# lukeduball/VoxelRaymarcher

Hardware: NVIDIA B200
Metric: primary_mrays_per_s_4k_512cube (higher is better)
Workload: dtype f32

## Files before the change

__graft_entry__.py:

```python
from __future__ import annotations

import os
import subprocess
import sys

ROOT = os.path.dirname(os.path.abspath(__file__))
if ROOT not in sys.path:
    sys.path.insert(0, ROOT)


def _run(cmd):
    proc = subprocess.run(cmd, cwd=ROOT, stdout=subprocess.PIPE, stderr=subprocess.STDOUT, text=True)
    if proc.returncode != 0:
        raise RuntimeError(f"{' '.join(cmd)} failed:\n{proc.stdout[-4000:]}")
    return proc.stdout


def build() -> None:
    _run(["make", "-j4", "-C", os.path.join(ROOT, "voxelraymarcher_b200", "csrc")])
    _run(["make", "-C", os.path.join(ROOT, "oracle"), "port"])
    _run(["make", "-j3", "-C", os.path.join(ROOT, "oracle"), "ref"])
    _run(["make", "-C", os.path.join(ROOT, "tests", "hostsim")])
    import voxelraymarcher_b200
    from voxelraymarcher_b200 import api
    api.load_library()


def smoke() -> None:
    import numpy as np
    from voxelraymarcher_b200 import api, scenes
    from oracle import pyoracle as po

    if not api.device_available():
        raise RuntimeError("smoke() needs a CUDA device: the product has no CPU fallback")
    xyz, rgb = scenes.probe_scene()
    width, height = 320, 180
    cam = api.Camera((6.0, 2.0, 6.0), (0.0, 0.0, -1.0), (0.0, 1.0, 0.0), 60.0, np.float32(width) / np.float32(height))
    kind = "refh" if po.available("refh") else "orc"
    po.set_lighting(kind)
    for storage in ("hashtable", "vcs"):
        scene = api.VoxelScene(0)
        scene.add_voxels(xyz, rgb)
        scene.generate_voxel_scene(storage)
        ref = po.OracleScene(kind)
        ref.add_voxels(xyz, rgb)
# ... 21 lines not shown
```

include/vrm_b200.h:

```cpp
#ifndef VRM_B200_H
#define VRM_B200_H

#include <stdint.h>

#ifdef __cplusplus
extern "C" {
#endif

typedef struct vrm_scene vrm_scene;

enum
{
	VRM_OK = 0,
	VRM_ERR_INVALID = 1,
	VRM_ERR_CUDA = 2,
	VRM_ERR_STATE = 3,
	VRM_ERR_NOMEM = 4,
	VRM_ERR_BUILD = 5
};

enum { VRM_STORAGE_VCS = 0, VRM_STORAGE_HASHTABLE = 1 };
enum { VRM_ALGO_LONGEST_AXIS = 0, VRM_ALGO_ORIGINAL = 1 };

#define VRM_EMPTY (1u << 30)
// ... 58 lines not shown

#define VRM_IPC_HANDLE_BYTES 64
int vrm_peer_alloc(int device, uint64_t bytes, void** d_ptr_out, unsigned char handle_out[VRM_IPC_HANDLE_BYTES]);
int vrm_peer_open(int device, const unsigned char handle[VRM_IPC_HANDLE_BYTES], void** d_ptr_out);
int vrm_peer_close(int device, void* d_ptr);
int vrm_peer_free(int device, void* d_ptr);
int vrm_copy_device(int device, void* d_dst, const void* d_src, uint64_t bytes);

int vrm_scene_set_completion_flag(vrm_scene* scene, uint32_t* d_flag, uint32_t first_value);
int vrm_scene_set_completion_counter(vrm_scene* scene, uint32_t* d_counter);
int vrm_claim_next(int device, void* cuda_stream, uint32_t* d_counter, uint32_t* h_claimed);
int vrm_wait_flags_device(int device, void* cuda_stream, const uint32_t* d_flags, uint32_t n_flags, uint32_t stride_words,
                          uint32_t min_value, uint32_t timeout_ms, int* d_status);

int vrm_render_views_sharded(vrm_scene* const* scenes, uint32_t n_scenes, const float* cameras, uint32_t n_views,
                             const float translation[3], uint32_t scale, int algorithm, uint32_t width, uint32_t height,
                             uint8_t* rgb_out, int out_on_device, uint32_t* views_per_scene_out, float* total_ms);

int vrm_lookup(vrm_scene* scene, const int32_t* xyz, uint64_t n, uint32_t* out, uint8_t* exists_out);

int vrm_set_l2_persistence(vrm_scene* scene, int enabled);

int vrm_set_statistics(vrm_scene* scene, int enabled);
int vrm_get_statistics(vrm_scene* scene, uint64_t out[8]);

int vrm_microbench_l2(int device, uint64_t working_set_bytes, float* gather8_loads_per_ns, float* gather8_gbs, float* stream_gbs);

#ifdef __cplusplus
}
#endif
#endif
```

voxelraymarcher_b200/api.py:

```python
from __future__ import annotations

import ctypes as C
import os

import numpy as np

HERE = os.path.dirname(os.path.abspath(__file__))
LIB_PATH = os.environ.get("VRM_B200_LIB") or os.path.join(HERE, "libvrm_b200.so")

STORAGE_VCS, STORAGE_HASHTABLE = 0, 1
ALGO_LONGEST_AXIS, ALGO_ORIGINAL = 0, 1
STORAGE = {"vcs": STORAGE_VCS, "hashtable": STORAGE_HASHTABLE}
ALGORITHM = {"longestaxis": ALGO_LONGEST_AXIS, "original": ALGO_ORIGINAL}
EMPTY = 1 << 30

EXPORTS = [
    "vrm_error_string", "vrm_last_error", "vrm_device_available", "vrm_device_count", "vrm_device_name", "vrm_scene_create", "vrm_scene_destroy",
    "vrm_scene_set_stream", "vrm_scene_reset_stream", "vrm_scene_synchronize", "vrm_scene_add_voxels", "vrm_scene_add_voxels_device", "vrm_scene_insert_voxel",
    "vrm_scene_generate_terrain", "vrm_scene_generate_sparse_shells", "vrm_scene_generate_cube", "vrm_scene_generate_sphere",
    "vrm_scene_build", "vrm_scene_info", "vrm_set_lighting", "vrm_camera_make", "vrm_make_unit_vector", "vrm_render",
    "vrm_render_device", "vrm_render_views_device", "vrm_render_views_device_strided", "vrm_render_views", "vrm_trace_rays", "vrm_trace_rays_device", "vrm_lookup",
    "vrm_set_l2_persistence", "vrm_set_statistics", "vrm_get_statistics", "vrm_peer_alloc", "vrm_peer_open", "vrm_peer_close", "vrm_peer_free", "vrm_copy_device", "vrm_microbench_l2",
    "vrm_scene_set_completion_flag", "vrm_scene_set_completion_counter", "vrm_claim_next", "vrm_wait_flags_device", "vrm_render_views_sharded",
]


class VrmError(RuntimeError):
    pass


_lib = None


def load_library():
    global _lib
    if _lib is not None:
        return _lib
    if not os.path.exists(LIB_PATH):
        raise VrmError(f"{LIB_PATH} is missing: build it with `python -c 'import __graft_entry__ as g; g.build()'` "
                       "(there is no CPU fallback)")
    lib = C.CDLL(LIB_PATH)
    vp, u64, u32, i32, ci, f32 = C.c_void_p, C.c_uint64, C.c_uint32, C.c_int32, C.c_int, C.c_float
    sig = {
        "vrm_error_string": (C.c_char_p, [ci]),
        "vrm_last_error": (C.c_char_p, [vp]),
# ... 12 lines not shown
        "vrm_scene_generate_sparse_shells": (ci, [vp, u32, u32, u32, u32, C.POINTER(u64)]),
        "vrm_scene_generate_cube": (ci, [vp, i32, i32, i32, i32, C.POINTER(u64)]),
        "vrm_scene_generate_sphere": (ci, [vp, u32, u32, u32, u32, ci, C.POINTER(u64)]),
        "vrm_scene_build": (ci, [vp, ci, C.POINTER(f32)]),
        "vrm_scene_info": (ci, [vp, C.POINTER(u32), C.POINTER(i32), C.POINTER(u32), C.POINTER(u64), C.POINTER(u64)]),
        "vrm_set_lighting": (ci, [vp, vp, vp, vp, ci, ci]),
        "vrm_camera_make": (ci, [vp, vp, vp, f32, f32, vp]),
        "vrm_make_unit_vector": (ci, [vp, vp]),
        "vrm_render": (ci, [vp, vp, vp, u32, ci, u32, u32, vp, vp, C.POINTER(f32)]),
        "vrm_render_device": (ci, [vp, vp, vp, u32, ci, u32, u32, vp, vp]),
        "vrm_render_views_device": (ci, [vp, vp, u32, vp, u32, ci, u32, u32, vp, vp]),
        "vrm_render_views_device_strided": (ci, [vp, vp, u32, vp, u32, ci, u32, u32, vp, vp, u32]),
        "vrm_render_views": (ci, [vp, vp, u32, vp, u32, ci, u32, u32, vp, C.POINTER(f32)]),
        "vrm_trace_rays": (ci, [vp, vp, u64, vp, u32, ci, vp, vp, C.POINTER(f32)]),
        "vrm_trace_rays_device": (ci, [vp, vp, u64, vp, u32, ci, vp, vp]),
        "vrm_lookup": (ci, [vp, vp, u64, vp, vp]),
        "vrm_peer_alloc": (ci, [ci, u64, C.POINTER(vp), vp]),
        "vrm_peer_open": (ci, [ci, vp, C.POINTER(vp)]),
        "vrm_peer_close": (ci, [ci, vp]),
        "vrm_peer_free": (ci, [ci, vp]),
        "vrm_copy_device": (ci, [ci, vp, vp, u64]),
        "vrm_set_l2_persistence": (ci, [vp, ci]),
        "vrm_set_statistics": (ci, [vp, ci]),
        "vrm_get_statistics": (ci, [vp, vp]),
        "vrm_microbench_l2": (ci, [ci, u64, C.POINTER(f32), C.POINTER(f32), C.POINTER(f32)]),
        "vrm_scene_set_completion_flag": (ci, [vp, vp, u32]),
        "vrm_scene_set_completion_counter": (ci, [vp, vp]),
        "vrm_claim_next": (ci, [ci, vp, vp, vp]),
        "vrm_wait_flags_device": (ci, [ci, vp, vp, u32, u32, u32, u32, vp]),
        "vrm_render_views_sharded": (ci, [vp, u32, vp, u32, vp, u32, ci, u32, u32, vp, ci, vp, C.POINTER(f32)]),
    }
    for name, (res, args) in sig.items():
        fn = getattr(lib, name)
        fn.restype = res
        fn.argtypes = args
    _lib = lib
    return lib


def device_available() -> bool:
    return bool(load_library().vrm_device_available())


def microbench_l2(device: int = 0, working_set_bytes: int = 32 << 20):
    a, b, c = C.c_float(), C.c_float(), C.c_float()
    rc = load_library().vrm_microbench_l2(device, working_set_bytes, C.byref(a), C.byref(b), C.byref(c))
# ... 196 lines not shown
                          translation=(0.0, 0.0, 0.0)):
        self._check(self.lib.vrm_trace_rays_device(self.h, C.c_void_p(d_rays_ptr), n, _ptr(_f3(translation)), scale, self._algo(algorithm),
                                                   C.c_void_p(d_colour_ptr), C.c_void_p(d_hits_ptr or 0)), "vrm_trace_rays_device")

    def lookup(self, xyz):
        xyz = np.ascontiguousarray(xyz, np.int32).reshape(-1, 3)
        n = xyz.shape[0]
        out = np.zeros(n, np.uint32)
        exists = np.zeros(n, np.uint8)
        self._check(self.lib.vrm_lookup(self.h, _ptr(xyz), n, _ptr(out), _ptr(exists)), "vrm_lookup")
        return out, exists

    def set_completion_flag(self, d_flag_ptr: int | None, first_value: int = 1):
        self._check(self.lib.vrm_scene_set_completion_flag(self.h, C.c_void_p(d_flag_ptr or 0), first_value), "vrm_scene_set_completion_flag")

    def set_completion_counter(self, d_counter_ptr: int | None):
        self._check(self.lib.vrm_scene_set_completion_counter(self.h, C.c_void_p(d_counter_ptr or 0)), "vrm_scene_set_completion_counter")

    def set_l2_persistence(self, enabled: bool):
        self._check(self.lib.vrm_set_l2_persistence(self.h, int(enabled)), "vrm_set_l2_persistence")

    def set_statistics(self, enabled: bool, as_executed: bool = False):
        self._check(self.lib.vrm_set_statistics(self.h, (2 if as_executed else 1) if enabled else 0), "vrm_set_statistics")

    def get_statistics(self):
        out = np.zeros(8, np.uint64)
        self._check(self.lib.vrm_get_statistics(self.h, _ptr(out)), "vrm_get_statistics")
        keys = ["exist_checks", "exist_false", "lookups", "lookup_hits", "table2_probes", "region_reads", "rays", "crawl_skipped"]
        return {k: int(v) for k, v in zip(keys, out)}


def render_views_sharded(scene_list, width, height, algorithm, cameras, scale=1, translation=(0.0, 0.0, 0.0), rgb_out=None, d_rgb_ptr: int | None = None):
    lib = load_library()
    cams = np.ascontiguousarray(np.stack([VoxelScene._cam(c) for c in cameras]).astype(np.float32))
    n = cams.shape[0]
    handles = (C.c_void_p * len(scene_list))(*[s.h for s in scene_list])
    counts = np.zeros(len(scene_list), np.uint32)
    ms = C.c_float()
    on_device = d_rgb_ptr is not None
    if not on_device:
        if rgb_out is None:
            rgb_out = np.zeros((n, height, width, 3), np.uint8)
        assert rgb_out.dtype == np.uint8 and rgb_out.size == n * height * width * 3 and rgb_out.flags["C_CONTIGUOUS"]
    out = C.c_void_p(d_rgb_ptr) if on_device else _ptr(rgb_out)
    rc = lib.vrm_render_views_sharded(C.cast(handles, C.c_void_p), len(scene_list), _ptr(cams), n, _ptr(_f3(translation)), int(scale),
                                      VoxelScene._algo(algorithm), width, height, out, int(on_device), _ptr(counts), C.byref(ms))
# ... 4 lines not shown
```

voxelraymarcher_b200/csrc/vrm_api.cu:

```cuda
#include "vrm_internal.h"
#include "../../include/vrm_b200.h"

#include <cmath>
#include <cstdlib>
#include <cstring>
#include <new>

using namespace vrm;

int vrm_fail_cuda(vrm_scene* s, cudaError_t e, const char* what)
{
	if (s) s->lastError = std::string(what) + ": " + cudaGetErrorString(e);
	cudaGetLastError();
	return e == cudaErrorMemoryAllocation ? VRM_ERR_NOMEM : VRM_ERR_CUDA;
}

void vrm_apply_l2_window(vrm_scene* s)
{
	const bool want = s->l2Persist && s->storage >= 0;
	if (want == s->l2WindowOn && (!want || s->l2WindowStream == s->stream)) return;
	cudaStreamAttrValue attr;
	memset(&attr, 0, sizeof(attr));
	if (s->l2WindowOn && s->l2WindowStream && s->l2WindowStream != s->stream)
	{
// ... 135 lines not shown
	s->device = device;
	float inv[3] = {1.0f, 1.0f, 1.0f};
	vrm_make_unit_vector(inv, s->light.dir);
	s->light.color[0] = s->light.color[1] = s->light.color[2] = 1.0f;
	s->light.pos[0] = 10.0f; s->light.pos[1] = 10.0f; s->light.pos[2] = -10.0f;
	s->light.usePoint = 0; s->light.useShadows = 1;
	cudaError_t e = cudaSetDevice(device);
	if (e == cudaSuccess) vrm_configure_pool(device);
	if (e == cudaSuccess) e = cudaStreamCreateWithFlags(&s->ownStream, cudaStreamNonBlocking);
	if (e == cudaSuccess) e = cudaEventCreate(&s->ev0);
	if (e == cudaSuccess) e = cudaEventCreate(&s->ev1);
	if (e == cudaSuccess) e = cudaMalloc(&s->d_stats, sizeof(Stats));
	if (e == cudaSuccess) e = cudaMemset(s->d_stats, 0, sizeof(Stats));
	if (e == cudaSuccess) e = cudaMalloc(&s->d_queue, sizeof(unsigned int));

	if (e == cudaSuccess) e = cudaDeviceGetAttribute(&s->numSms, cudaDevAttrMultiProcessorCount, device);
	if (const char* mode = getenv("VRM_RENDER_MODE")) s->renderMode = atoi(mode);
	if (const char* form = getenv("VRM_SHADOW_FORM")) { const int f = atoi(form); if (f >= 0 && f <= 2) s->shadowForm = f; }
	if (const char* lp = getenv("VRM_L2_PERSIST")) s->l2Persist = atoi(lp) != 0;
	if (const char* ts = getenv("VRM_TRACE_SORT")) s->traceSort = atoi(ts);
	if (const char* tf = getenv("VRM_TRACE_FUSED")) s->traceFused = atoi(tf);
	if (const char* pd = getenv("VRM_PINNED_DMA")) s->pinnedDma = atoi(pd);
	if (const char* ws = getenv("VRM_WSTORE_REMOTE")) s->wstoreRemote = atoi(ws) != 0;
	if (const char* bs = getenv("VRM_BULK_STORE")) s->bulkStore = atoi(bs) != 0;
	if (const char* bb = getenv("VRM_VIEW_BATCH_BYTES")) { long long v = atoll(bb); if (v > 0) s->viewBatchBytes = (size_t)v; }
	if (e != cudaSuccess) { vrm_scene_destroy(s); cudaGetLastError(); return VRM_ERR_CUDA; }
	s->stream = s->ownStream;
	cudaEventRecord(s->ev1, s->stream);
	*out = s;
	return VRM_OK;
}

int vrm_scene_destroy(vrm_scene* s)
{
	if (!s) return VRM_OK;
	cudaSetDevice(s->device);
	if (s->stream) cudaStreamSynchronize(s->stream);
	vrm_stage_free(s);
	vrm_free_async(s, s->d_regionMinMax); s->d_regionMinMax = nullptr;
	vrm_free_structure(s);
	cudaStreamSynchronize(s->stream);
	cudaFree(s->d_hits); cudaFree(s->d_cams); cudaFree(s->d_io); cudaFree(s->d_stats); cudaFree(s->d_queue); cudaFree(s->d_defer); cudaFree(s->d_parkBits); cudaFree(s->d_parkCtl); cudaFree(s->d_gather); cudaFree(s->d_shadowItems); cudaFree(s->d_shadowCtl); cudaFree(s->d_localFrame); if (s->h_stage) cudaFreeHost(s->h_stage); for (auto& e : s->evBand) if (e) cudaEventDestroy(e);
	if (s->h_cams) cudaFreeHost(s->h_cams);
	if (s->ev0) cudaEventDestroy(s->ev0);
	if (s->ev1) cudaEventDestroy(s->ev1);
	if (s->ownStream) cudaStreamDestroy(s->ownStream);
// ... 421 lines not shown
{
	if (!d_dst || !d_src) return VRM_ERR_INVALID;
	if (cudaSetDevice(device) != cudaSuccess || cudaMemcpy(d_dst, d_src, bytes, cudaMemcpyDeviceToDevice) != cudaSuccess) { cudaGetLastError(); return VRM_ERR_CUDA; }
	return VRM_OK;
}

int vrm_set_l2_persistence(vrm_scene* s, int enabled)
{
	if (!s) return VRM_ERR_INVALID;
	VRM_CUDA(s, cudaSetDevice(s->device));
	s->l2Persist = enabled != 0;
	vrm_apply_l2_window(s);
	return VRM_OK;
}

int vrm_set_statistics(vrm_scene* s, int enabled)
{
	if (!s) return VRM_ERR_INVALID;
	s->statsEnabled = enabled != 0;
	s->statsMode = enabled == 2 ? 2 : (enabled ? 1 : 0);
	return VRM_OK;
}

int vrm_get_statistics(vrm_scene* s, uint64_t out[8])
{
	if (!s || !out) return VRM_ERR_INVALID;
	VRM_CUDA(s, cudaSetDevice(s->device));
	Stats h;
	VRM_CUDA(s, cudaMemcpyAsync(&h, s->d_stats, sizeof(Stats), cudaMemcpyDeviceToHost, s->stream));
	VRM_CUDA(s, cudaStreamSynchronize(s->stream));
	out[0] = h.nExist; out[1] = h.nExistFalse; out[2] = h.nLookup; out[3] = h.nLookupHit; out[4] = h.nProbe2; out[5] = h.nRegionReads;
	out[6] = s->statsRays; out[7] = h.nCrawlSkipped;
	return VRM_OK;
}

}
```

voxelraymarcher_b200/csrc/vrm_build.cu:

```cuda
#include "vrm_internal.h"

#include <chrono>
#include <cstdio>
#include <cstdlib>
#include "../../include/vrm_b200.h"

#include <algorithm>

using namespace vrm;

namespace
{

constexpr int kThreads = 256;
constexpr int kSortItems = 8;
constexpr int kSortTile = kThreads * kSortItems;
constexpr int kMaxDigitBits = 9;
constexpr int kMaxBins = 1 << kMaxDigitBits;
constexpr int kScanItems = 8;
constexpr int kScanTile = kThreads * kScanItems;
constexpr int kMaxEvictions = 400;
constexpr int kMaxRebuilds = 24;
constexpr int kRoundsPerBatch = 3;

// ... 190 lines not shown
	cellOcc[cell] = 1u;
}

__global__ void counts_kernel(const uint32_t* __restrict__ pos, const uint32_t* __restrict__ keep, uint64_t n,
                              const uint32_t* __restrict__ cellRank, const uint32_t* __restrict__ cellOcc, uint64_t cells, uint32_t* __restrict__ counts)
{
	counts[0] = pos[n - 1] + keep[n - 1];
	counts[1] = cellRank[cells - 1] + cellOcc[cells - 1];
}

__global__ void region_table_kernel(const uint32_t* __restrict__ cellFirst, const uint32_t* __restrict__ cellRank, const uint32_t* __restrict__ cellOcc, uint64_t cells,
                                    uint32_t numRegions, uint32_t unique, int32_t* __restrict__ regionTable, uint32_t* __restrict__ regionStart)
{
	uint64_t c = blockIdx.x * (uint64_t)blockDim.x + threadIdx.x;
	if (c == 0) regionStart[numRegions] = unique;
	if (c >= cells) return;
	if (cellOcc[c])
	{
		const uint32_t ri = cellRank[c];
		regionTable[c] = (int32_t)ri;
		regionStart[ri] = cellFirst[c];
	}
	else regionTable[c] = -1;
}

template <class K>
__global__ void vcs_fill_kernel(const K* __restrict__ ukeys, const int32_t* __restrict__ regionTable, uint64_t u,
                                uint2* __restrict__ headers, uint32_t* __restrict__ clusterMask)
{
	uint64_t j = blockIdx.x * (uint64_t)blockDim.x + threadIdx.x;
	if (j >= u) return;
	K k = ukeys[j];
	if (j != 0 && (ukeys[j - 1] >> 5) == (k >> 5)) return;
	uint32_t ri = (uint32_t)regionTable[(uint64_t)(k >> 18)];
	uint32_t cid = (uint32_t)(k >> 9) & 511u, code = (uint32_t)k & 511u;
	uint32_t mask = 1u << (code & 31);
	for (uint64_t t = j + 1; t < u && t < j + 32; t++)
	{
		K kt = ukeys[t];
		if ((kt >> 5) != (k >> 5)) break;
		mask |= 1u << ((uint32_t)kt & 31);
	}
	headers[((size_t)ri * 512 + cid) * 16 + (code >> 5)] = make_uint2(mask, (uint32_t)j);
	bool firstOfCluster = j == 0 || (ukeys[j - 1] >> 9) != (k >> 9);
	if (firstOfCluster) atomicOr(clusterMask + (size_t)ri * 16 + (cid >> 5), 1u << (cid & 31));
}
// ... 186 lines not shown
		region_heads_kernel<K><<<grid_for(n), kThreads, 0, st>>>(kin, pos, n, cellFirst, cellOcc);
		exclusive_scan(cellOcc, cellRank, tableSize, scratch, st);
		counts_kernel<<<1, 1, 0, st>>>(pos, keep, n, cellRank, cellOcc, tableSize, counts);
		uint32_t hostCounts[2] = {0, 0};
		VRM_CUDA(s, cudaMemcpyAsync(hostCounts, counts, sizeof(hostCounts), cudaMemcpyDeviceToHost, st));
		VRM_CUDA(s, cudaStreamSynchronize(st));
		unique = hostCounts[0];
		numRegions = hostCounts[1];
		if (unique == n) { ukeys = kin; uvals = vin; valsAreStageRgb = vin == s->d_stageRgb; }
		else
		{
			if (uniq.alloc(pad256(unique * sizeof(K)) + unique * 4) != cudaSuccess) { cudaGetLastError(); s->lastError = "unique voxel allocation failed"; return VRM_ERR_NOMEM; }
			ukeys = uniq.as<K>();
			uvals = reinterpret_cast<uint32_t*>(uniq.as<char>() + pad256(unique * sizeof(K)));
			compact_kernel<K><<<grid_for(n), kThreads, 0, st>>>(kin, vin, keep, pos, n, ukeys, uvals);
		}
		trace.mark(st, "dedupe + region heads");
		if (regionStart.alloc(((size_t)numRegions + 1) * 4) != cudaSuccess) { cudaGetLastError(); s->lastError = "region directory allocation failed"; return VRM_ERR_NOMEM; }
		region_table_kernel<<<grid_for(tableSize), kThreads, 0, st>>>(cellFirst, cellRank, cellOcc, tableSize, numRegions, (uint32_t)unique, regionTable.as<int32_t>(), regionStart.as<uint32_t>());
		VRM_CUDA(s, cudaGetLastError());
		trace.mark(st, "region directory");
	}

	uint64_t bytes = tableSize * sizeof(int32_t);
	PoolBuf headers(s), clusterMask(s), hashDesc(s), slots(s), values(s);
	if (storageType == VRM_STORAGE_VCS)
	{
		constexpr size_t kGuardClusters = 80;
		const size_t headerGuard = kGuardClusters * 16 * sizeof(uint2), maskGuard = 128;
		const size_t headerBytes = (size_t)numRegions * 512 * 16 * sizeof(uint2);
		if (unique >= (1ull << 31) || ((uint64_t)numRegions * 512ull + kGuardClusters) * 16ull >= (1ull << 32)) { s->lastError = "scene too large for the VCS index widths"; return VRM_ERR_INVALID; }
		if (headers.alloc(headerBytes + headerGuard) != cudaSuccess || clusterMask.alloc((size_t)numRegions * 16 * 4 + maskGuard) != cudaSuccess)
		{ cudaGetLastError(); s->lastError = "VCS allocation failed"; return VRM_ERR_NOMEM; }
		VRM_CUDA(s, cudaMemsetAsync(headers.p, 0, headerBytes + headerGuard, st));
		VRM_CUDA(s, cudaMemsetAsync(clusterMask.p, 0, (size_t)numRegions * 16 * 4 + maskGuard, st));
		if (unique)
		{
			vcs_fill_kernel<K><<<grid_for(unique), kThreads, 0, st>>>(ukeys, regionTable.as<int32_t>(), unique, headers.as<uint2>(), clusterMask.as<uint32_t>());
			vcs_flag_clusters_kernel<<<grid_for((uint64_t)numRegions * 512), kThreads, 0, st>>>(headers.as<uint2>(), clusterMask.as<uint32_t>(), (uint64_t)numRegions * 512);
		}
		if (unique && valsAreStageRgb) { values.s = s; values.p = s->d_stageRgb; s->d_stageRgb = nullptr; }
		else
		{
			if (values.alloc(unique * 4) != cudaSuccess) { cudaGetLastError(); s->lastError = "colour array allocation failed"; return VRM_ERR_NOMEM; }
			if (unique) VRM_CUDA(s, cudaMemcpyAsync(values.p, uvals, unique * 4, cudaMemcpyDeviceToDevice, st));
		}
		VRM_CUDA(s, cudaGetLastError());
// ... 31 lines not shown
				for (; round < batchEnd; round++)
				{
					cuckoo_insert_kernel<K><<<grid_for(unique), kThreads, 0, st>>>(ukeys, uvals, regionTable.as<int32_t>(), unique, hashDesc.as<HashRegionDesc>(),
					                                                              slots.as<unsigned long long>(), retry, failed, failCount, round);
					cuckoo_round_end_kernel<<<numRegions, kThreads, 0, st>>>(slots.as<unsigned long long>(), hashDesc.as<HashRegionDesc>(), retry, failed, failCount, round);
				}
				uint32_t hostFail[kMaxRebuilds] = {};
				VRM_CUDA(s, cudaMemcpyAsync(hostFail, failCount, round * 4, cudaMemcpyDeviceToHost, st));
				VRM_CUDA(s, cudaStreamSynchronize(st));
				for (uint32_t r = 0; r < round; r++) if (hostFail[r] == 0u) converged = true;
				if (trace.on) for (uint32_t r = 0; r < round; r++) fprintf(stderr, "[vrm build] cuckoo round %u: %u regions failed\n", r, hostFail[r]);
			}
			if (!converged) { s->lastError = "cuckoo insertion did not converge"; return VRM_ERR_BUILD; }
			VRM_CUDA(s, cudaGetLastError());
		}
		bytes += (size_t)numRegions * sizeof(HashRegionDesc) + totalSlots * 8 + (size_t)numRegions * 64;
		trace.mark(st, "cuckoo insertion");
	}
	VRM_CUDA(s, cudaEventRecord(s->ev1, st));
	VRM_CUDA(s, cudaStreamSynchronize(st));
	VRM_CUDA(s, cudaGetLastError());

	s->d_regionTable = static_cast<int32_t*>(regionTable.release());
	if (storageType == VRM_STORAGE_VCS)
	{
		s->d_headers = static_cast<uint2*>(headers.release());
		s->d_clusterMask = static_cast<uint32_t*>(clusterMask.release());
		s->d_values = static_cast<uint32_t*>(values.release());
	}
	else
	{
		s->d_hashDesc = static_cast<HashRegionDesc*>(hashDesc.release());
		s->d_clusterMask = static_cast<uint32_t*>(clusterMask.release());
		s->d_slots = static_cast<unsigned long long*>(slots.release());
	}
	s->storage = storageType;
	s->diameter = (uint32_t)D;
	s->minCoord = minCoord;
	s->filled = numRegions;
	s->unique = unique;
	s->bytes = bytes;
	return VRM_OK;
}

}

// ... 63 lines not shown
	*d_xyz = s->d_stageXyz + s->nStaged * 3;
	*d_rgb = s->d_stageRgb + s->nStaged;
	return VRM_OK;
}

int vrm_stage_commit(vrm_scene* s, uint64_t n)
{
	if (n == 0) return VRM_OK;
	if (!s->d_regionMinMax)
	{
		cudaError_t e = vrm_alloc_async(s, reinterpret_cast<void**>(&s->d_regionMinMax), 2 * sizeof(int));
		if (e == cudaSuccess) e = cudaMemsetAsync(s->d_regionMinMax, 0, 2 * sizeof(int), s->stream);
		if (e != cudaSuccess) return vrm_fail_cuda(s, e, "region extent allocation");
	}
	region_minmax_kernel<<<(unsigned)std::min<uint64_t>((n * 3 + kThreads - 1) / kThreads, 148 * 16), kThreads, 0, s->stream>>>(s->d_stageXyz + s->nStaged * 3, n, s->d_regionMinMax);
	VRM_CUDA(s, cudaGetLastError());
	s->nStaged += n;
	return VRM_OK;
}

void vrm_free_structure(vrm_scene* s)
{
	vrm_free_async(s, s->d_regionTable); s->d_regionTable = nullptr;
	vrm_free_async(s, s->d_hashDesc); s->d_hashDesc = nullptr;
	vrm_free_async(s, s->d_slots); s->d_slots = nullptr;
	vrm_free_async(s, s->d_headers); s->d_headers = nullptr;
	vrm_free_async(s, s->d_clusterMask); s->d_clusterMask = nullptr;
	vrm_free_async(s, s->d_values); s->d_values = nullptr;
	s->storage = -1; s->bytes = 0; s->filled = 0; s->unique = 0;
}

int vrm_build_structure(vrm_scene* s, int storageType, float* buildMs)
{
	cudaStream_t st = s->stream;
	BuildTrace trace;
	VRM_CUDA(s, cudaEventRecord(s->ev0, st));
	int rc = vrm_stage_flush_pending(s);
	if (rc) return rc;
	int hostMinMax[2] = {0, 0};
	if (s->d_regionMinMax)
	{
		VRM_CUDA(s, cudaMemcpyAsync(hostMinMax, s->d_regionMinMax, sizeof(hostMinMax), cudaMemcpyDeviceToHost, st));
		VRM_CUDA(s, cudaStreamSynchronize(st));
	}
	trace.mark(st, "extent");
	const int minCoord = hostMinMax[0];
// ... 46 lines not shown
```

voxelraymarcher_b200/csrc/vrm_core.cuh:

```cuda
#pragma once

#ifndef VRM_SMEM_MASK
#define VRM_SMEM_MASK 0
#endif

#include <stdint.h>
#include <math.h>
#include <string.h>
#include <type_traits>

#if defined(__CUDACC__)
#define VRM_HD __host__ __device__ __forceinline__
#define VRM_HD_NOINLINE static __host__ __device__ __noinline__
#else
#define VRM_HD inline
#define VRM_HD_NOINLINE static inline
#endif

namespace vrm
{

constexpr float kEps = 0.0001f;
constexpr uint32_t kEmpty = 1u << 30;
constexpr uint32_t kContinue = kEmpty + 2u;
// ... 106 lines not shown

VRM_HD float div1(float x, const RayDir& k, int i)
{
	float ax = fabsf(x);
	if (!(ax >= k.thr)) return vdiv(x, k.d[i]);
	return div_by_const(x, k.d[i], k.rd[i]);
}


struct Lighting
{
	float dir[3];
	float color[3];
	float pos[3];
	int usePoint;
	int useShadows;
};

struct LightWalk
{
	float idD[3], idR[3], idThr;
	float laD[3], laR[3], laSD[3], laSR[3], laThr;
	uint32_t laPerm;
};

struct HashRegionDesc
{
	uint32_t slotBase;
	uint32_t n;
	uint32_t seed1, seed2;
};

struct SceneView
{
	const int32_t* regionTable;
	uint32_t diameter;
	int32_t minCoord;
	const HashRegionDesc* hashDesc;
	const unsigned long long* slots;
	const uint2* headers;
	const uint32_t* clusterMask;
	const uint32_t* values;
};

struct Stats
{
	unsigned long long nExist, nExistFalse, nLookup, nLookupHit, nProbe2, nRegionReads;
	unsigned long long nCrawlSkipped;
};


struct PermIdentity
{
	VRM_HD int axis(int i) const { return i; }
	VRM_HD int cs(int i) const { return 6 - 3 * i; }
	VRM_HD int ks(int i) const { return 14 - 7 * i; }
	VRM_HD uint32_t stride(int i, uint32_t D) const { return i == 0 ? 1u : (i == 1 ? D : D * D); }
};
// ... 208 lines not shown
	if (STATS) c.st.nLookup++;
	if (v != kEmpty) note_lookup_hit(c, p, reg, g0, g1, g2);
	return v;
}

template <int ST, bool STATS, class P>
VRM_HD void record_hit_voxel(RayCtx<ST, STATS>& c, const P& p, const int* reg, int g0, int g1, int g2)
{
	if (!c.hitOut) return;
	int gw[3] = {reg[0] * kRegion + g0, reg[1] * kRegion + g1, reg[2] * kRegion + g2};
	int gx[3];
	to_world(p, gw, gx);
	c.hitOut[0] = gx[0]; c.hitOut[1] = gx[1]; c.hitOut[2] = gx[2]; c.hitOut[3] = 1;
}

template <int ST, bool STATS, class P>
VRM_HD int32_t region_entry(RayCtx<ST, STATS>& c, const P& p, const int* reg)
{
	uint32_t D = c.sv.diameter;
	uint32_t u0 = (uint32_t)(reg[0] - c.sv.minCoord), u1 = (uint32_t)(reg[1] - c.sv.minCoord), u2 = (uint32_t)(reg[2] - c.sv.minCoord);
	if (!(u0 < D && u1 < D && u2 < D)) return -2;
	if (STATS) c.st.nRegionReads++;
	return ldg(c.sv.regionTable + (u0 * p.stride(0, D) + u1 * p.stride(1, D) + u2 * p.stride(2, D)));
}


VRM_HD uint32_t vec_to_rgb(float r, float g, float b)
{
	uint32_t ir = (uint32_t)vmul(r, 255.0f), ig = (uint32_t)vmul(g, 255.0f), ib = (uint32_t)vmul(b, 255.0f);
	return (ir << 16) | (ig << 8) | ib;
}

VRM_HD uint32_t apply_lighting(const Lighting& L, const float* translation, uint32_t voxelColor, int normalAxis, float normalSign,
                               const float* hitLocal, const int* regW)
{
	float cr = vdiv((float)(voxelColor >> 16), 255.0f);
	float cg = vdiv((float)((voxelColor >> 8) & 0xFF), 255.0f);
	float cb = vdiv((float)(voxelColor & 0xFF), 255.0f);
	float n[3] = {0.0f, 0.0f, 0.0f};
	n[0] = normalAxis == 0 ? normalSign : 0.0f;
	n[1] = normalAxis == 1 ? normalSign : 0.0f;
	n[2] = normalAxis == 2 ? normalSign : 0.0f;
	if (L.usePoint)
	{
		float t[3];
		for (int i = 0; i < 3; i++)
// ... 580 lines not shown
```

voxelraymarcher_b200/csrc/vrm_flat.cuh:

```cuda
#pragma once

#include "vrm_core.cuh"

#if defined(__CUDACC__)
#define VRM_FLAT_COLD __host__ __device__ __noinline__
#else
#define VRM_FLAT_COLD
#endif

#ifndef VRM_VCS_FUSED_EXIST
#define VRM_VCS_FUSED_EXIST 1
#endif

namespace vrm
{

enum FlatState : int
{
	kStMainLast = 4,
	kStRegion = 5,
	kStHead = 6,
	kStHit = 7,
	kStDone = 8,
	kStPark = 9
};

enum AdvMode : int
{
	kAdvNone = 0,
	kAdvNext = 1,
	kAdvCluster = 2,
	kAdvJump = 3,
	kAdvRegion = 4
};

constexpr uint32_t kFlShadow = 1u;
constexpr uint32_t kFlShadowLA = 2u;
constexpr uint32_t kFlEq0 = 4u;
constexpr uint32_t kFlEqMask = 28u;
constexpr int kFlPermShift = 8;
constexpr int32_t kRiPending = -3;

constexpr int kPpOff = 0, kPpDefer = 1, kPpInline = 2;
#ifndef VRM_REGION_VOTE
#define VRM_REGION_VOTE 0
#endif
#ifndef VRM_HEAD_VOTE
#define VRM_HEAD_VOTE 0
#endif
#ifndef VRM_PP_DEFAULT
#define VRM_PP_DEFAULT 2
#endif
#ifndef VRM_FAST_LA
#define VRM_FAST_LA 7
#endif
#ifndef VRM_CC_MUL
#define VRM_CC_MUL 1
#endif
#ifndef VRM_CLS_LUT
#define VRM_CLS_LUT 1
#endif
#ifndef VRM_FAST_ENTER
// ... 16 lines not shown

VRM_HD PermRuntime unpack_perm(uint32_t fl)
{
	PermRuntime p;
	p.a0 = (int)((fl >> kFlPermShift) & 3u); p.a1 = (int)((fl >> (kFlPermShift + 2)) & 3u); p.a2 = (int)((fl >> (kFlPermShift + 4)) & 3u);
	return p;
}
VRM_HD uint32_t pack_perm(const PermRuntime& p) { return ((uint32_t)p.a0 | ((uint32_t)p.a1 << 2) | ((uint32_t)p.a2 << 4)) << kFlPermShift; }

VRM_HD LightWalk make_light_walk(const Lighting& L)
{
	LightWalk w;
	const RayDir ki = make_raydir(L.dir[0], L.dir[1], L.dir[2]);
	for (int i = 0; i < 3; i++) { w.idD[i] = ki.d[i]; w.idR[i] = ki.rd[i]; }
	w.idThr = ki.thr;
	const PermRuntime p = rank_axes(L.dir[0], L.dir[1], L.dir[2]);
	float dw[3];
	to_walk(p, L.dir, dw);
	const RayDir k = make_raydir(dw[0], dw[1], dw[2]);
	const RayDir ko = scaled_raydir(k);
	for (int i = 0; i < 3; i++) { w.laD[i] = k.d[i]; w.laR[i] = k.rd[i]; w.laSD[i] = ko.d[i]; w.laSR[i] = ko.rd[i]; }
	w.laThr = (k.thr == k.thr && ko.thr == ko.thr) ? k.thr : NAN;
	w.laPerm = pack_perm(p);
	return w;
}

VRM_HD uint32_t apply_lighting_flat(const Lighting& L, const float* translation, uint32_t voxelColor, int normalAxis, float normalSign,
                                    const float* hitLocal, const int* regW)
{
	if (L.usePoint) return apply_lighting(L, translation, voxelColor, normalAxis, normalSign, hitLocal, regW);
	const float r255 = 0.00392156886f;
	const float cr = div_by_const((float)(voxelColor >> 16), 255.0f, r255);
	const float cg = div_by_const((float)((voxelColor >> 8) & 0xFF), 255.0f, r255);
	const float cb = div_by_const((float)(voxelColor & 0xFF), 255.0f, r255);
	const float n0 = normalAxis == 0 ? normalSign : 0.0f, n1 = normalAxis == 1 ? normalSign : 0.0f, n2 = normalAxis == 2 ? normalSign : 0.0f;
	const float diff = fmaxf(vadd(vadd(vmul(n0, L.dir[0]), vmul(n1, L.dir[1])), vmul(n2, L.dir[2])), 0.0f);
	return vec_to_rgb(vmul(cr, vmul(diff, L.color[0])), vmul(cg, vmul(diff, L.color[1])), vmul(cb, vmul(diff, L.color[2])));
}

VRM_HD void primary_ray_flat(const float* cam, uint32_t x, uint32_t y, uint32_t W, uint32_t H, float invW, float invH, float* o, float* d)
{
	const float u = div_by_const(vadd((float)x, 0.5f), (float)W, invW);
	const float v = div_by_const(vadd((float)(H - y), 0.5f), (float)H, invH);
	float rel[3];
	for (int i = 0; i < 3; i++)
	{
// ... 37 lines not shown
		st = kStDone;
	}

	VRM_HD void set_perm(const SceneView& sv, const PermRuntime& p)
	{
		fl = (fl & ~(63u << kFlPermShift)) | pack_perm(p);
		const uint32_t D = sv.diameter;
		const int a[3] = {p.a0, p.a1, p.a2};
		for (int i = 0; i < 3; i++)
		{
			sh[i] = ST == kStorageHash ? (uint32_t)(kHashKeyBits * (2 - a[i])) : (uint32_t)(6 - 3 * a[i]);
#if VRM_CC_MUL
			sh[i] = 1u << sh[i];
#endif
			rs[i] = a[i] == 0 ? 1u : (a[i] == 1 ? D : D * D);
		}
	}

	VRM_HD void read_region_entry(RayCtx<ST, STATS>& c)
	{
		const uint32_t D = c.sv.diameter;
		if (!(ur[0] < D && ur[1] < D && ur[2] < D)) { ri = -2; return; }
		if (STATS) c.st.nRegionReads++;
		ri = ldg(c.sv.regionTable + (ur[0] * rs[0] + ur[1] * rs[1] + ur[2] * rs[2]));
	}

	VRM_HD void change_region(RayCtx<ST, STATS>& c)
	{
		for (int i = 0; i < 3; i++)
		{
			const int diff = (int)floorf(vmul(o[i], 0.015625f));
			ur[i] += (uint32_t)diff;
			o[i] = vsub(o[i], (float)(diff * kRegion));
		}
		st = kStRegion;
		if (!position_sane(o)) { ri = -2; return; }
		read_region_entry(c);
	}

	VRM_HD void start_primary(RayCtx<ST, STATS>& c, const float* originW, const float* dirW, float scale)
	{
		fl = 0; result = 0; ri = -2; seq = 0; ad1 = ad2 = 0;
		g[0] = g[1] = g[2] = 0; ro[0] = ro[1] = ro[2] = 0.0f;
		PermRuntime p;
		p.a0 = 0; p.a1 = 1; p.a2 = 2;
		if constexpr (kLA) p = rank_axes(dirW[0], dirW[1], dirW[2]);
		set_perm(c.sv, p);
		float sW[3] = {canonical_zero(vmul(scale, vsub(originW[0], c.translation[0]))), canonical_zero(vmul(scale, vsub(originW[1], c.translation[1]))),
		               canonical_zero(vmul(scale, vsub(originW[2], c.translation[2])))};
		float dw[3];
		to_walk(p, sW, o); to_walk(p, dirW, dw);
		const RayDir k = make_raydir(dw[0], dw[1], dw[2]);
		for (int i = 0; i < 3; i++) { d[i] = k.d[i]; rd[i] = k.rd[i]; }
		thr = k.thr;
		if constexpr (kLA)
		{
			const RayDir ko = scaled_raydir(k);
			for (int i = 0; i < 3; i++) { sd[i] = ko.d[i]; srd[i] = ko.rd[i]; }
			if (!(ko.thr == ko.thr)) thr = NAN;
		}
		int reg[3] = {(int)floorf(vmul(o[0], 0.015625f)), (int)floorf(vmul(o[1], 0.015625f)), (int)floorf(vmul(o[2], 0.015625f))};
		const int minC = c.sv.minCoord;
		const uint32_t D = c.sv.diameter;
		while (reg[0] - minC < 0 || reg[1] - minC < 0 || reg[2] - minC < 0 ||
		       (uint32_t)(reg[0] - minC) > D - 1 || (uint32_t)(reg[1] - minC) > D - 1 || (uint32_t)(reg[2] - minC) > D - 1)
// ... 32 lines not shown
		}
		result = col;
		ro[0] = p0; ro[1] = p1; ro[2] = p2;
		seq = (uint32_t)(nAxisW | (nSign < 0.0f ? 4 : 0) | (laKind ? 8 : 0));
		st = kStHit;
	}

	VRM_HD void shade_hit(RayCtx<ST, STATS>& c, ShadowStart& ss) const
	{
		const int nAxisW = (int)(seq & 3u);
		const float nSign = (seq & 4u) ? -1.0f : 1.0f;
		const PermRuntime p = unpack_perm(fl);
		const int minC = c.sv.minCoord;
		const int reg[3] = {(int)ur[0] + minC, (int)ur[1] + minC, (int)ur[2] + minC};
		to_world(p, ro, ss.hitW); to_world(p, reg, ss.regW);
		ss.lit = apply_lighting_flat(c.light, c.translation, result, nAxisW, nSign, ss.hitW, ss.regW);
		ss.la = (kLA && (seq & 8u) != 0) ? 1 : 0;
	}

	VRM_HD void start_shadow(RayCtx<ST, STATS>& c, const ShadowStart& ss)
	{
		const bool laKind = kLA && ss.la != 0;
		result = ss.lit;
		fl = kFlShadow | (laKind ? kFlShadowLA : 0u);
		seq = 0; ad1 = ad2 = 0; ri = -2;
		g[0] = g[1] = g[2] = 0; ro[0] = ro[1] = ro[2] = 0.0f;
		PermRuntime p;
		p.a0 = 0; p.a1 = 1; p.a2 = 2;
		if (laKind) p = unpack_perm(c.lw.laPerm);
		set_perm(c.sv, p);
		to_walk(p, ss.hitW, o);
		{
			int regWalk[3];
			to_walk(p, ss.regW, regWalk);
			const int minC = c.sv.minCoord;
			for (int i = 0; i < 3; i++) ur[i] = (uint32_t)(regWalk[i] - minC);
		}
		if (laKind)
		{
			for (int i = 0; i < 3; i++) { d[i] = c.lw.laD[i]; rd[i] = c.lw.laR[i]; }
			if constexpr (kLA) { for (int i = 0; i < 3; i++) { sd[i] = c.lw.laSD[i]; srd[i] = c.lw.laSR[i]; } }
			thr = c.lw.laThr;
		}
		else
		{
			for (int i = 0; i < 3; i++) { d[i] = c.lw.idD[i]; rd[i] = c.lw.idR[i]; }
			thr = c.lw.idThr;
// ... 701 lines not shown
```

voxelraymarcher_b200/csrc/vrm_internal.h:

```cpp
#pragma once

#include <cuda_runtime.h>
#include <stdint.h>
#include <string>
#include <vector>

#include "vrm_core.cuh"

constexpr uint64_t kPendingFlushVoxels = 1ull << 20;
constexpr uint64_t kPendingMaxCall = 1ull << 14;

struct vrm_scene
{
	int device = 0;
	cudaStream_t ownStream = nullptr;
	cudaStream_t stream = nullptr;
	std::string lastError;

	int32_t* d_stageXyz = nullptr;
	uint32_t* d_stageRgb = nullptr;
	uint64_t stageCap = 0;
	uint64_t nStaged = 0;
	int* d_regionMinMax = nullptr;
	std::vector<int32_t> pendingXyz;
	std::vector<uint32_t> pendingRgb;

	int storage = -1;
	uint32_t diameter = 0;
	int32_t minCoord = 0;
	uint32_t filled = 0;
	uint64_t unique = 0;
	uint64_t bytes = 0;
	int32_t* d_regionTable = nullptr;
	vrm::HashRegionDesc* d_hashDesc = nullptr;
	unsigned long long* d_slots = nullptr;
	uint2* d_headers = nullptr;
	uint32_t* d_clusterMask = nullptr;
	uint32_t* d_values = nullptr;

	vrm::Lighting light;

	int32_t* d_hits = nullptr;   size_t hitsBytes = 0;
	float* d_cams = nullptr;     size_t camsBytes = 0;
	float* h_cams = nullptr;
	void* d_io = nullptr;        size_t ioBytes = 0;
	cudaEvent_t ev0 = nullptr, ev1 = nullptr;
	uint8_t* h_stage = nullptr;  size_t stageBytes = 0;
	cudaEvent_t evBand[8] = {};
	cudaStream_t copyStream = nullptr;
	cudaEvent_t evRendered[2] = {nullptr, nullptr}, evCopied[2] = {nullptr, nullptr};
	uint8_t* d_batch[2] = {nullptr, nullptr};  size_t batchBytes = 0;
	size_t viewBatchBytes = size_t(256) << 20;

	unsigned int* d_queue = nullptr;
	void* d_defer = nullptr;
	uint32_t* d_parkBits = nullptr;   size_t parkWords = 0;
// ... 1 lines not shown
	int numSms = 148;
	int renderMode = -1;

	bool l2Persist = false;
	cudaStream_t l2WindowStream = nullptr;
	bool l2WindowOn = false;

	uint32_t* d_doneFlag = nullptr;
	uint32_t doneSeq = 0;
	uint32_t* d_doneCounter = nullptr;
	uint8_t* d_gather = nullptr;      size_t gatherBytes = 0;

	void* d_shadowItems = nullptr;    size_t shadowCap = 0;
	unsigned int* d_shadowCtl = nullptr;

	uint8_t* d_dmaFrame = nullptr;    size_t dmaFrameBytes = 0;
	int pinnedDma = 0;
	int traceSort = 1;
	int traceFused = 1;
	bool bulkStore = true;
	bool wstoreRemote = false;
	uint8_t* d_localFrame = nullptr;  size_t localFrameBytes = 0;
	int shadowForm = -1;
	int statsMode = 0;
	bool statsEnabled = false;
	vrm::Stats* d_stats = nullptr;
	uint64_t statsRays = 0;

	vrm::SceneView view() const
	{
		vrm::SceneView v;
		v.regionTable = d_regionTable; v.diameter = diameter; v.minCoord = minCoord;
		v.hashDesc = d_hashDesc; v.slots = d_slots;
		v.headers = d_headers; v.clusterMask = d_clusterMask; v.values = d_values;
		return v;
	}
};

int vrm_fail_cuda(vrm_scene* s, cudaError_t e, const char* what);
#define VRM_CUDA(s, call)                                                   \
	do {                                                                    \
		cudaError_t e__ = (call);                                           \
		if (e__ != cudaSuccess) return vrm_fail_cuda((s), e__, #call);      \
	} while (0)

int vrm_build_structure(vrm_scene* s, int storageType, float* buildMs);
void vrm_free_structure(vrm_scene* s);
int vrm_stage_reserve(vrm_scene* s, uint64_t extra, int32_t** d_xyz, uint32_t** d_rgb);
int vrm_stage_commit(vrm_scene* s, uint64_t n);
int vrm_stage_flush_pending(vrm_scene* s);
void vrm_stage_free(vrm_scene* s);
cudaError_t vrm_alloc_async(vrm_scene* s, void** p, size_t bytes);
void vrm_free_async(vrm_scene* s, void* p);
void vrm_configure_pool(int device);
size_t vrm_scan_scratch_elems(uint64_t n);
// ... 15 lines not shown
```

Before: 6819.

## Add per-octant exit-ahead table to terminate rays early in empty space

```diff
diff --git a/__graft_entry__.py b/__graft_entry__.py
--- a/__graft_entry__.py
+++ b/__graft_entry__.py
@@ -21,6 +21,9 @@
     _run(["make", "-C", os.path.join(ROOT, "oracle"), "port"])
     _run(["make", "-j3", "-C", os.path.join(ROOT, "oracle"), "ref"])
     _run(["make", "-C", os.path.join(ROOT, "tests", "hostsim")])
+    hs = os.path.join(ROOT, "tests", "hostsim")
+    _run(["g++", "-std=c++17", "-O2", "-ffp-contract=off", "-fPIC", "-shared", "-fopenmp", os.path.join(hs, "exit_ahead_sim.cpp"),
+          "-o", os.path.join(hs, "libexitsim.so")])
     import voxelraymarcher_b200
     from voxelraymarcher_b200 import api
     api.load_library()
diff --git a/include/vrm_b200.h b/include/vrm_b200.h
--- a/include/vrm_b200.h
+++ b/include/vrm_b200.h
@@ -104,6 +104,7 @@
 int vrm_set_l2_persistence(vrm_scene* scene, int enabled);
 
 int vrm_set_statistics(vrm_scene* scene, int enabled);
+int vrm_set_exit_ahead(vrm_scene* scene, int enabled);
 int vrm_get_statistics(vrm_scene* scene, uint64_t out[8]);
 
 int vrm_microbench_l2(int device, uint64_t working_set_bytes, float* gather8_loads_per_ns, float* gather8_gbs, float* stream_gbs);
diff --git a/voxelraymarcher_b200/api.py b/voxelraymarcher_b200/api.py
--- a/voxelraymarcher_b200/api.py
+++ b/voxelraymarcher_b200/api.py
@@ -20,7 +20,7 @@
     "vrm_scene_generate_terrain", "vrm_scene_generate_sparse_shells", "vrm_scene_generate_cube", "vrm_scene_generate_sphere",
     "vrm_scene_build", "vrm_scene_info", "vrm_set_lighting", "vrm_camera_make", "vrm_make_unit_vector", "vrm_render",
     "vrm_render_device", "vrm_render_views_device", "vrm_render_views_device_strided", "vrm_render_views", "vrm_trace_rays", "vrm_trace_rays_device", "vrm_lookup",
-    "vrm_set_l2_persistence", "vrm_set_statistics", "vrm_get_statistics", "vrm_peer_alloc", "vrm_peer_open", "vrm_peer_close", "vrm_peer_free", "vrm_copy_device", "vrm_microbench_l2",
+    "vrm_set_l2_persistence", "vrm_set_statistics", "vrm_set_exit_ahead", "vrm_get_statistics", "vrm_peer_alloc", "vrm_peer_open", "vrm_peer_close", "vrm_peer_free", "vrm_copy_device", "vrm_microbench_l2",
     "vrm_scene_set_completion_flag", "vrm_scene_set_completion_counter", "vrm_claim_next", "vrm_wait_flags_device", "vrm_render_views_sharded",
 ]
 
@@ -79,6 +79,7 @@
         "vrm_copy_device": (ci, [ci, vp, vp, u64]),
         "vrm_set_l2_persistence": (ci, [vp, ci]),
         "vrm_set_statistics": (ci, [vp, ci]),
+        "vrm_set_exit_ahead": (ci, [vp, ci]),
         "vrm_get_statistics": (ci, [vp, vp]),
         "vrm_microbench_l2": (ci, [ci, u64, C.POINTER(f32), C.POINTER(f32), C.POINTER(f32)]),
         "vrm_scene_set_completion_flag": (ci, [vp, vp, u32]),
@@ -321,6 +322,9 @@
 
     def set_statistics(self, enabled: bool, as_executed: bool = False):
         self._check(self.lib.vrm_set_statistics(self.h, (2 if as_executed else 1) if enabled else 0), "vrm_set_statistics")
+
+    def set_exit_ahead(self, enabled: bool):
+        self._check(self.lib.vrm_set_exit_ahead(self.h, int(enabled)), "vrm_set_exit_ahead")
 
     def get_statistics(self):
         out = np.zeros(8, np.uint64)
diff --git a/voxelraymarcher_b200/csrc/vrm_api.cu b/voxelraymarcher_b200/csrc/vrm_api.cu
--- a/voxelraymarcher_b200/csrc/vrm_api.cu
+++ b/voxelraymarcher_b200/csrc/vrm_api.cu
@@ -181,6 +181,7 @@
 	if (const char* tf = getenv("VRM_TRACE_FUSED")) s->traceFused = atoi(tf);
 	if (const char* pd = getenv("VRM_PINNED_DMA")) s->pinnedDma = atoi(pd);
 	if (const char* ws = getenv("VRM_WSTORE_REMOTE")) s->wstoreRemote = atoi(ws) != 0;
+	if (const char* ea = getenv("VRM_EXIT_AHEAD")) s->exitAhead = atoi(ea) != 0;
 	if (const char* bs = getenv("VRM_BULK_STORE")) s->bulkStore = atoi(bs) != 0;
 	if (const char* bb = getenv("VRM_VIEW_BATCH_BYTES")) { long long v = atoll(bb); if (v > 0) s->viewBatchBytes = (size_t)v; }
 	if (e != cudaSuccess) { vrm_scene_destroy(s); cudaGetLastError(); return VRM_ERR_CUDA; }
@@ -648,6 +649,13 @@
 	return VRM_OK;
 }
 
+int vrm_set_exit_ahead(vrm_scene* s, int enabled)
+{
+	if (!s) return VRM_ERR_INVALID;
+	s->exitAhead = enabled != 0;
+	return VRM_OK;
+}
+
 int vrm_get_statistics(vrm_scene* s, uint64_t out[8])
 {
 	if (!s || !out) return VRM_ERR_INVALID;
diff --git a/voxelraymarcher_b200/csrc/vrm_build.cu b/voxelraymarcher_b200/csrc/vrm_build.cu
--- a/voxelraymarcher_b200/csrc/vrm_build.cu
+++ b/voxelraymarcher_b200/csrc/vrm_build.cu
@@ -236,6 +236,12 @@
 		regionStart[ri] = cellFirst[c];
 	}
 	else regionTable[c] = -1;
+}
+
+__global__ void exit_ahead_kernel(const int32_t* __restrict__ regionTable, uint8_t* __restrict__ t, uint32_t D, int axis)
+{
+	const uint64_t line = blockIdx.x * (uint64_t)blockDim.x + threadIdx.x;
+	if (line < (uint64_t)D * D) exit_ahead_line(regionTable, t, D, axis, (uint32_t)line);
 }
 
 template <class K>
@@ -468,7 +474,14 @@
 		trace.mark(st, "region directory");
 	}
 
-	uint64_t bytes = tableSize * sizeof(int32_t);
+	PoolBuf exitAhead(s);
+	if (exitAhead.alloc(2 * tableSize) != cudaSuccess) { cudaGetLastError(); s->lastError = "region table allocation failed"; return VRM_ERR_NOMEM; }
+	VRM_CUDA(s, cudaMemsetAsync(exitAhead.as<uint8_t>() + tableSize, 0, tableSize, st));
+	for (int axis = 0; axis < 3; axis++) exit_ahead_kernel<<<grid_for(D * D), kThreads, 0, st>>>(regionTable.as<int32_t>(), exitAhead.as<uint8_t>(), (uint32_t)D, axis);
+	VRM_CUDA(s, cudaGetLastError());
+	trace.mark(st, "exit-ahead table");
+
+	uint64_t bytes = tableSize * (sizeof(int32_t) + 1);
 	PoolBuf headers(s), clusterMask(s), hashDesc(s), slots(s), values(s);
 	if (storageType == VRM_STORAGE_VCS)
 	{
@@ -546,6 +559,8 @@
 	VRM_CUDA(s, cudaGetLastError());
 
 	s->d_regionTable = static_cast<int32_t*>(regionTable.release());
+	s->d_exitAhead = exitAhead.as<uint8_t>();
+	exitAhead.release();
 	if (storageType == VRM_STORAGE_VCS)
 	{
 		s->d_headers = static_cast<uint2*>(headers.release());
@@ -655,6 +670,7 @@
 void vrm_free_structure(vrm_scene* s)
 {
 	vrm_free_async(s, s->d_regionTable); s->d_regionTable = nullptr;
+	vrm_free_async(s, s->d_exitAhead); s->d_exitAhead = nullptr;
 	vrm_free_async(s, s->d_hashDesc); s->d_hashDesc = nullptr;
 	vrm_free_async(s, s->d_slots); s->d_slots = nullptr;
 	vrm_free_async(s, s->d_headers); s->d_headers = nullptr;
diff --git a/voxelraymarcher_b200/csrc/vrm_core.cuh b/voxelraymarcher_b200/csrc/vrm_core.cuh
--- a/voxelraymarcher_b200/csrc/vrm_core.cuh
+++ b/voxelraymarcher_b200/csrc/vrm_core.cuh
@@ -152,7 +152,13 @@
 	float idD[3], idR[3], idThr;
 	float laD[3], laR[3], laSD[3], laSR[3], laThr;
 	uint32_t laPerm;
-};
+	uint32_t octFl;
+};
+
+VRM_HD uint32_t exit_octant(float dx, float dy, float dz)
+{
+	return (dx < 0.0f ? 1u : 0u) | (dy < 0.0f ? 2u : 0u) | (dz < 0.0f ? 4u : 0u);
+}
 
 struct HashRegionDesc
 {
@@ -164,6 +170,7 @@
 struct SceneView
 {
 	const int32_t* regionTable;
+	const uint8_t* exitAhead = nullptr;
 	uint32_t diameter;
 	int32_t minCoord;
 	const HashRegionDesc* hashDesc;
@@ -418,6 +425,31 @@
 	if (!(u0 < D && u1 < D && u2 < D)) return -2;
 	if (STATS) c.st.nRegionReads++;
 	return ldg(c.sv.regionTable + (u0 * p.stride(0, D) + u1 * p.stride(1, D) + u2 * p.stride(2, D)));
+}
+
+VRM_HD void exit_ahead_line(const int32_t* regionTable, uint8_t* t, uint32_t D, int axis, uint32_t line)
+{
+	const uint32_t a = line % D, b = line / D;
+	const uint32_t stride = axis == 0 ? 1u : (axis == 1 ? D : D * D);
+	const uint32_t base = axis == 0 ? a * D + b * D * D : (axis == 1 ? a + b * D * D : a + b * D);
+	const uint32_t neg = axis == 0 ? 0xAAu : (axis == 1 ? 0xCCu : 0xF0u);
+	uint32_t acc = 0u;
+	for (uint32_t i = 0; i < D; i++)
+	{
+		const uint32_t cell = base + i * stride;
+		const uint32_t v = axis == 0 ? (regionTable[cell] >= 0 ? 0xFFu : 0u) : (uint32_t)t[cell];
+		acc |= v;
+		t[cell] = (uint8_t)((acc & neg) | (v & ~neg));
+	}
+	acc = 0u;
+	for (uint32_t i = D; i-- > 0;)
+	{
+		const uint32_t cell = base + i * stride;
+		const uint32_t v = t[cell];
+		acc |= v & ~neg;
+		const uint32_t r = (v & neg) | acc;
+		t[cell] = (uint8_t)(axis == 2 ? ~r : r);
+	}
 }
 
 
diff --git a/voxelraymarcher_b200/csrc/vrm_flat.cuh b/voxelraymarcher_b200/csrc/vrm_flat.cuh
--- a/voxelraymarcher_b200/csrc/vrm_flat.cuh
+++ b/voxelraymarcher_b200/csrc/vrm_flat.cuh
@@ -38,6 +38,7 @@
 constexpr uint32_t kFlShadowLA = 2u;
 constexpr uint32_t kFlEq0 = 4u;
 constexpr uint32_t kFlEqMask = 28u;
+constexpr int kFlOctShift = 5;
 constexpr int kFlPermShift = 8;
 constexpr int32_t kRiPending = -3;
 
@@ -100,6 +101,7 @@
 	for (int i = 0; i < 3; i++) { w.laD[i] = k.d[i]; w.laR[i] = k.rd[i]; w.laSD[i] = ko.d[i]; w.laSR[i] = ko.rd[i]; }
 	w.laThr = (k.thr == k.thr && ko.thr == ko.thr) ? k.thr : NAN;
 	w.laPerm = pack_perm(p);
+	w.octFl = exit_octant(L.dir[0], L.dir[1], L.dir[2]) << kFlOctShift;
 	return w;
 }
 
@@ -183,7 +185,18 @@
 		const uint32_t D = c.sv.diameter;
 		if (!(ur[0] < D && ur[1] < D && ur[2] < D)) { ri = -2; return; }
 		if (STATS) c.st.nRegionReads++;
-		ri = ldg(c.sv.regionTable + (ur[0] * rs[0] + ur[1] * rs[1] + ur[2] * rs[2]));
+		const uint32_t cell = ur[0] * rs[0] + ur[1] * rs[1] + ur[2] * rs[2];
+		ri = ldg(c.sv.regionTable + cell);
+#if defined(__CUDA_ARCH__)
+		const uint32_t ahead = ldg(c.sv.exitAhead + cell);
+#else
+		const uint32_t ahead = c.sv.exitAhead ? (uint32_t)c.sv.exitAhead[cell] : 0u;
+#endif
+		if (ri == -1 && ((ahead >> ((fl >> kFlOctShift) & 7u)) & 1u) != 0u && fmaxf(o[0], fmaxf(o[1], o[2])) < 64.0f)
+		{
+			ri = -2;
+			st = kStDone;
+		}
 	}
 
 	VRM_HD void change_region(RayCtx<ST, STATS>& c)
@@ -201,7 +214,7 @@
 
 	VRM_HD void start_primary(RayCtx<ST, STATS>& c, const float* originW, const float* dirW, float scale)
 	{
-		fl = 0; result = 0; ri = -2; seq = 0; ad1 = ad2 = 0;
+		fl = exit_octant(dirW[0], dirW[1], dirW[2]) << kFlOctShift; result = 0; ri = -2; seq = 0; ad1 = ad2 = 0;
 		g[0] = g[1] = g[2] = 0; ro[0] = ro[1] = ro[2] = 0.0f;
 		PermRuntime p;
 		p.a0 = 0; p.a1 = 1; p.a2 = 2;
@@ -280,7 +293,7 @@
 	{
 		const bool laKind = kLA && ss.la != 0;
 		result = ss.lit;
-		fl = kFlShadow | (laKind ? kFlShadowLA : 0u);
+		fl = kFlShadow | (laKind ? kFlShadowLA : 0u) | c.lw.octFl;
 		seq = 0; ad1 = ad2 = 0; ri = -2;
 		g[0] = g[1] = g[2] = 0; ro[0] = ro[1] = ro[2] = 0.0f;
 		PermRuntime p;
diff --git a/voxelraymarcher_b200/csrc/vrm_internal.h b/voxelraymarcher_b200/csrc/vrm_internal.h
--- a/voxelraymarcher_b200/csrc/vrm_internal.h
+++ b/voxelraymarcher_b200/csrc/vrm_internal.h
@@ -32,6 +32,7 @@
 	uint64_t unique = 0;
 	uint64_t bytes = 0;
 	int32_t* d_regionTable = nullptr;
+	uint8_t* d_exitAhead = nullptr;
 	vrm::HashRegionDesc* d_hashDesc = nullptr;
 	unsigned long long* d_slots = nullptr;
 	uint2* d_headers = nullptr;
@@ -79,6 +80,7 @@
 	bool wstoreRemote = false;
 	uint8_t* d_localFrame = nullptr;  size_t localFrameBytes = 0;
 	int shadowForm = -1;
+	bool exitAhead = true;
 	int statsMode = 0;
 	bool statsEnabled = false;
 	vrm::Stats* d_stats = nullptr;
@@ -88,6 +90,7 @@
 	{
 		vrm::SceneView v;
 		v.regionTable = d_regionTable; v.diameter = diameter; v.minCoord = minCoord;
+		v.exitAhead = d_exitAhead ? d_exitAhead + ((exitAhead && statsMode != 1) ? 0 : (size_t)diameter * diameter * diameter) : nullptr;
 		v.hashDesc = d_hashDesc; v.slots = d_slots;
 		v.headers = d_headers; v.clusterMask = d_clusterMask; v.values = d_values;
 		return v;
```

After: 6969 (median of 6 runs). 2.2% higher.
